# marcinp7/music-style-transfer

Measured on AMD Instinct MI355X. Metric: style-transfer opt iters/sec, higher is better.
Workload: dtype f32; 1 GPU; one 30 s clip per GPU (BASELINE.json configs[1]): piano-roll C=4,R=16,T=4 (+percussion), full widths (980325 params), fwd+loss+bwd every step, Adam+StepLR every iter_size steps; clips_per_gpu=1, iter_size=2, hip_graph=True, graphs=one joint graph, accumulation=2 concurrent streams, launches_per_pass=71, parallelism=single GPU

## Files before the change

include/mst_amd.h:

```cpp
#ifndef MST_AMD_H
#define MST_AMD_H
#include <stdint.h>

#ifdef __cplusplus
extern "C" {
#endif

typedef enum {
    MST_OK = 0,
    MST_ERR_ARG = -1,
    MST_ERR_UNSUPPORTED = -2,
    MST_ERR_LAUNCH = -3,
    MST_ERR_ALLOC = -4,
} mst_status;

typedef struct {
    int32_t C, R, T;
    int32_t beat, bar, nrf;
    int32_t style, melody, rhythm;
    int32_t instr;
    int32_t n_instruments;
    int32_t has_unpitched;
    int32_t clips;
} mst_dims;
// ... 6 lines not shown
    MST_L_U_TOTAL, MST_L_U_NOTES, MST_L_U_VELOCITY, MST_L_U_DURATION,
    MST_L_SI_TOTAL, MST_L_SI_INSTRUMENTS, MST_L_SI_MODE, MST_L_SI_BPM,
    MST_N_LOSSES
};

typedef struct mst_plan mst_plan;
typedef void* mst_stream;

int32_t mst_param_count(const mst_dims* d);
int64_t mst_param_floats(const mst_dims* d);
int32_t mst_param_info(const mst_dims* d, int32_t i, char* name, int32_t name_cap,
                       int64_t* offset, int32_t* ndim, int32_t shape[3]);

int32_t mst_widths_supported(const mst_dims* d);

typedef struct {
    int32_t gemm_tile;
    int32_t no_merge;
    int32_t gemm_run;
    int32_t tile_r0, tile_rows;
    int32_t lstm_flavour;
    int32_t dense_flavour;
    int32_t branches;
} mst_plan_options;
mst_plan* mst_plan_create(const mst_dims* d, int32_t* status);
mst_plan* mst_plan_create_ex(const mst_dims* d, const mst_plan_options* opt, int32_t* status);
int32_t mst_plan_gemm_tile(const mst_plan* p);
void mst_plan_destroy(mst_plan* p);
int64_t mst_plan_workspace_floats(const mst_plan* p);
int32_t mst_plan_tensor(const mst_plan* p, const char* name, int64_t* off, int64_t* goff, int64_t* numel);
int32_t mst_plan_launch_count(const mst_plan* p, int32_t stage_mask, int32_t backward);
int32_t mst_plan_layout(const mst_plan* p, int64_t out[4]);

enum { MST_DEV_OK = 0, MST_DEV_LSTM_TIMEOUT = 1  };
int32_t mst_plan_status(const mst_plan* p, float* ws, int32_t clear, int32_t* status, mst_stream stream);

int32_t mst_forward(const mst_plan* p, int32_t stage_mask, const float* params, float* ws,
                    const float* pitched, const float* unpitched, mst_stream stream);

int32_t mst_backward(const mst_plan* p, int32_t stage_mask, const float* params, float* gparams,
                     float* ws, const float* pitched, const float* unpitched, mst_stream stream);
int32_t mst_zero_grads(const mst_plan* p, int32_t stage_mask, float* ws, mst_stream stream);
int64_t mst_plan_zero_floats(const mst_plan* p, int32_t stage_mask);

#define MST_LOSS_SAVED 512
int64_t mst_loss_scratch_floats(void);
// ... 80 lines not shown

int32_t mst_plan_step_count(const mst_plan* p, int32_t stage_mask, int32_t backward);
int32_t mst_plan_step_info(const mst_plan* p, int32_t stage_mask, int32_t backward, int32_t* info );
int32_t mst_plan_step_carried(const mst_plan* p, int32_t stage_mask, int32_t backward, int32_t* carried);
int32_t mst_plan_step_riders(const mst_plan* p, int32_t stage_mask, int32_t backward, int32_t* out);
int32_t mst_plan_zero_rides(const mst_plan* p);
int32_t mst_plan_step_carrier(const mst_plan* p, int32_t stage_mask, int32_t backward, int32_t* out);
int32_t mst_plan_set_lstm_small(mst_plan* p, int32_t on);
int32_t mst_plan_step_gemms(const mst_plan* p, int32_t stage_mask, int32_t backward, int32_t step, int32_t* out, int32_t cap);
int32_t mst_plan_time_steps(const mst_plan* p, int32_t stage_mask, int32_t backward, const float* params,
                            float* gparams, float* ws, const float* pitched, const float* unpitched,
                            mst_stream stream, int32_t reps, float* ms, int32_t* kind, double* flops, double* bytes);

typedef struct mst_audio_plan mst_audio_plan;
mst_audio_plan* mst_audio_plan_create(int32_t n_fft , int32_t hop, int64_t n_samples, int32_t* status);
void mst_audio_plan_destroy(mst_audio_plan* p);
int32_t mst_audio_plan_info(const mst_audio_plan* p, int64_t out[6]);
int32_t mst_audio_stft(const mst_audio_plan* p, const float* audio, float* spec, float* mag, mst_stream stream);
int32_t mst_audio_gram(const mst_audio_plan* p, const float* feat, float* gram, float* ws, mst_stream stream);
int32_t mst_audio_style_iteration(const mst_audio_plan* p, float* x, const float* gram_style, float* grad, float* exp_avg,
                                  float* exp_avg_sq, float* state, float* ws, float* loss, double lr, mst_stream stream);

int32_t mst_debug_slab_columns_disjoint(int64_t off_x, int32_t width_x, int64_t off_y, int32_t width_y, int32_t ld);
int64_t mst_debug_gemm_walk(int32_t kind, int32_t as_b, int32_t rows, int32_t K, int32_t k0, int32_t k1, int32_t kd, int32_t ld,
                            int32_t pb, int32_t pc, int32_t oc, int64_t* compared);
int32_t mst_plan_step_gemm_kinds(const mst_plan* p, int32_t stage_mask, int32_t backward, int32_t step, int32_t* out, int32_t cap);

const char* mst_version(void);

#ifdef __cplusplus
}
#endif
#endif
```

music-style-transfer_amd/csrc/gemm.hip:

```cpp
#include "combine_body.h"
#include "lstm_small_body.h"

__device__ __forceinline__ float act_fwd(int act, float z, int col) {
    if (act == ACT_LEAKY) return z > 0.f ? z : z * LEAKY;
    if (act == ACT_SIGOUT) { float s = 1.f / (1.f + expf(-z)); return col == 0 ? 6.f * s : s; }
    if (act == ACT_BPM) { float s = 1.f / (1.f + expf(-z)); return s * 150.f + 50.f; }
    return z;
}

__device__ __forceinline__ float act_bwd(int act, float y, int col) {
    if (act == ACT_LEAKY) return y > 0.f ? 1.f : LEAKY;
    if (act == ACT_SIGOUT) return col == 0 ? y * (1.f - y * (1.f / 6.f)) : y * (1.f - y);
    if (act == ACT_BPM) { float s = (y - 50.f) * (1.f / 150.f); return 150.f * s * (1.f - s); }
    return 1.f;
}

typedef const MST_GLOBAL_AS float* gcptr;
#define GEMM_PAD 1

template <int KIND>
__host__ __device__ __forceinline__ int off_of(const Operand& o, int i, int j, bool& ok) {
    if constexpr (KIND == OPK_DENSE) {
        return i * (int)o.si + j * (int)o.sj;
    } else if constexpr (KIND == OPK_ACTGRAD) {
// ... 154 lines not shown
    if (compared) *compared = seen;
    return bad;
}

extern "C" int64_t mst_debug_gemm_walk(int32_t kind, int32_t as_b, int32_t rows, int32_t K, int32_t k0, int32_t k1, int32_t kd,
                                       int32_t ld, int32_t pb, int32_t pc, int32_t oc, int64_t* compared) {
    if (rows < 1 || K < 1 || k0 < 0 || k0 % 8 || k1 > K || k0 > k1 || (kd != 32 && kd != 64 && kd != 128)) return MST_ERR_ARG;
    Operand o{};
    o.kind = kind; o.ld = ld; o.pb = pb; o.pc = pc; o.oc = oc; o.ones_at = -1;
#define WALK_KD(KIND, ISB, KF, PERM)                                                                      \
    return kd == 32 ? walk_mismatches<KIND, ISB, KF, 32, PERM>(o, rows, k0, k1, compared)                 \
                    : (kd == 64 ? walk_mismatches<KIND, ISB, KF, 64, PERM>(o, rows, k0, k1, compared)     \
                                : walk_mismatches<KIND, ISB, KF, 128, PERM>(o, rows, k0, k1, compared));
    if (kind == OPK_IM2COL && !as_b) { WALK_KD(OPK_IM2COL, false, 1, 0) }
    if (kind == OPK_IM2COL && as_b) { WALK_KD(OPK_IM2COL, true, 0, 0) }
    if (kind == OPK_CONVGRAD && !as_b) { WALK_KD(OPK_CONVGRAD, false, 1, 0) }
    if (kind == OPK_PERMW && as_b && perm_case(pb, pc) == 1) { WALK_KD(OPK_PERMW, true, 1, 1) }
    if (kind == OPK_PERMW && as_b && perm_case(pb, pc) == 2) { WALK_KD(OPK_PERMW, true, 1, 2) }
#undef WALK_KD
    return MST_ERR_UNSUPPORTED;
}

template <int OK>
__device__ __forceinline__ void store_out(const GemmDesc& d, float* cbase, const float* bias, int m, int n, int split, float acc) {
    const OutSpec& o = d.out;
    if constexpr (OK == OUT_STORE) {
        float v = acc;
        if (bias) v += o.bias_div > 0 ? bias[(unsigned)((m / o.bias_div) * o.bias_ld + n)] : bias[n];
        cbase[(unsigned)(m * o.ldc + n)] = act_fwd(o.act, v, n);
    } else if constexpr (OK == OUT_ACCUM) {
        float* c = cbase + (unsigned)(m * o.ldc + n);
        *c = o.first ? acc : *c + acc;
    } else if constexpr (OK == OUT_CONV) {
        cbase[(unsigned)((m >> 3) * o.ldc + n * NOCT + (m & 7))] = act_fwd(ACT_LEAKY, acc + bias[n], 0);
    } else if constexpr (OK == OUT_SLAB) {
        const unsigned idx = n < o.wcols ? (unsigned)(m * o.wcols + n) : (unsigned)(d.M * o.wcols + m);
        cbase[(int64_t)split * o.slab_stride + idx] = acc;
    } else {
        unsigned idx;
        if (n < o.wcols) {
            int a, bb, c, bc;
            if (o.pb == CONV_K && o.pc == NPF) { bc = CONV_K * NPF; a = n / (CONV_K * NPF); const int rem = n - a * (CONV_K * NPF); bb = rem / NPF; c = rem - bb * NPF; }
            else if (o.pb == NUN && o.pc == NUF) { bc = NUN * NUF; a = n / (NUN * NUF); const int rem = n - a * (NUN * NUF); bb = rem / NUF; c = rem - bb * NUF; }
            else { bc = o.pb * o.pc; a = n / bc; const int rem = n - a * bc; bb = rem / o.pc; c = rem - bb * o.pc; }
            idx = (unsigned)(m * o.wcols + a * bc + c * o.pb + bb);
        } else {
            idx = (unsigned)(d.M * o.wcols + m);
        }
        cbase[(int64_t)split * o.slab_stride + idx] = acc;
    }
}

template <int AK, int BKIND, int OK, int AKF, int BKF, int KD, int PERM = 0>
__device__ __forceinline__ void gemm_body(const GemmDesc& d, const Bases& b, const int tile, const int split,
                                          float (*As)[GEMM_BM + GEMM_PAD], float (*Bs)[GEMM_BN + GEMM_PAD]) {
    const int tid = threadIdx.x;
    const int M = d.M, N = d.N;
    const int tiles_n = (N + GEMM_BN - 1) / GEMM_BN;
    const gcptr baseA = (gcptr)(b.p[d.A.space] + d.A.off);
    const gcptr baseA2 = (AK == OPK_ACTGRAD || AK == OPK_CONVGRAD) ? (gcptr)(b.p[d.A.space2] + d.A.off2) : baseA;
    const gcptr baseB = (gcptr)(b.p[d.B.space] + d.B.off);
    const int tm = tile / tiles_n, tn = tile - tm * tiles_n;
    int kchunk = (d.K + d.ksplit - 1) / d.ksplit;
    kchunk = (kchunk + KD - 1) / KD * KD;
    const int k0 = split * kchunk;
    const int k1 = min(d.K, k0 + kchunk);
    const int wv = tid >> 6, lane = tid & 63;
    const int a_act = (AK == OPK_ACTGRAD) ? d.A.act : ACT_LEAKY;
    const int a_tr = d.A.transposed;
    const int b_ones = (BKIND == OPK_DENSE || BKIND == OPK_IM2COL) ? d.B.ones_at : -1;
    typedef float acc_f32x16 __attribute__((ext_vector_type(16)));
// ... 21 lines not shown
            int ia = wa.at(d.A, i, (KT), k1, ina, oka);                                                    \
            ia = oka ? ia : 0;                                                                             \
            const float x = baseA[(unsigned)ia];                                                           \
            if constexpr (AK == OPK_ACTGRAD || AK == OPK_CONVGRAD) {                                       \
                const float y = baseA2[(unsigned)ia];                                                      \
                int col = 0;                                                                               \
                if constexpr (AK == OPK_ACTGRAD) col = a_tr ? tm * GEMM_BM + A_ROW(i) : (KT) + A_KL(i);    \
                ya[i] = act_bwd(a_act, y, col);                                                            \
            } else ya[i] = 1.f;                                                                            \
            va[i] = oka ? x : 0.f;                                                                         \
            bool inb, okb;                                                                                 \
            int ib = wb.at(d.B, i, (KT), k1, inb, okb);                                                    \
            bool one = false;                                                                              \
            if constexpr (BKIND == OPK_DENSE || BKIND == OPK_IM2COL) one = inb & (tn * GEMM_BN + B_ROW(i) == b_ones); \
            ib = (okb & !one) ? ib : 0;                                                                    \
            const float w = baseB[(unsigned)ib];                                                           \
            vb[i] = one ? 1.f : (okb ? w : 0.f);                                                           \
        }                                                                                                  \
        wa.advance();                                                                                      \
        wb.advance();                                                                                      \
    }

    if (k0 < k1) GEMM_ISSUE(k0)
    for (int kt = k0; kt < k1; kt += KD) {
#pragma unroll
        for (int i = 0; i < NL; ++i) {
            As[A_KL(i)][A_ROW(i)] = (AK == OPK_ACTGRAD || AK == OPK_CONVGRAD) ? va[i] * ya[i] : va[i];
            Bs[B_KL(i)][B_ROW(i)] = vb[i];
        }
        __syncthreads();
        if (kt + KD < k1) GEMM_ISSUE(kt + KD)
#pragma unroll
        for (int kk = 0; kk < KW; kk += 2) {
            const int k = wv * KW + kk + (lane >> 5);
            acc = __builtin_amdgcn_mfma_f32_32x32x2f32(As[k][lane & 31], Bs[k][lane & 31], acc, 0, 0, 0);
        }
        __syncthreads();
    }
#undef GEMM_ISSUE
#undef A_ROW
#undef A_KL
#undef B_ROW
#undef B_KL
    float* red = &As[0][0];
#pragma unroll
    for (int r = 0; r < 16; ++r)
        red[wv * (GEMM_BM * GEMM_BN) + ((r & 3) + 8 * (r >> 2) + 4 * (lane >> 5)) * GEMM_BN + (lane & 31)] = acc[r];
    __syncthreads();
    float* cbase = b.p[d.out.space] + d.out.off;
    const float* bias = d.out.bias_space >= 0 ? b.p[d.out.bias_space] + d.out.bias_off : nullptr;
#pragma unroll
    for (int q = 0; q < GEMM_BM * GEMM_BN / NT; ++q) {
        const int o = tid + q * NT;
        const int m = tm * GEMM_BM + o / GEMM_BN, n = tn * GEMM_BN + o % GEMM_BN;
        float v = 0.f;
#pragma unroll
        for (int w = 0; w < NW; ++w) v += red[w * (GEMM_BM * GEMM_BN) + o];
        if (m < M && n < N) store_out<OK>(d, cbase, bias, m, n, split, v);
    }
}

#define MF_BM 64
#define MF_BN 64
#define MF_KD 32
#define MF_THREADS 256
typedef float mf_f32x16 __attribute__((ext_vector_type(16)));
typedef float mf_f4u __attribute__((ext_vector_type(4), aligned(4)));

template <int AK, int BKIND, int OK, int AKF, int BKF, bool FOLD = false>
__device__ __forceinline__ void gemm_mfma_body(const GemmDesc& d, const Bases& b, const int tile, const int split,
                                               float (*As)[MF_BM + GEMM_PAD], float (*Bs)[MF_BN + GEMM_PAD]) {
    const int tid = threadIdx.x;
    const int M = d.M, N = d.N;
    const int tiles_n = (N + MF_BN - 1) / MF_BN;
    const gcptr baseA = (gcptr)(b.p[d.A.space] + d.A.off);
    const gcptr baseA2 = (AK == OPK_ACTGRAD || AK == OPK_CONVGRAD) ? (gcptr)(b.p[d.A.space2] + d.A.off2) : baseA;
    const gcptr baseB = (gcptr)(b.p[d.B.space] + d.B.off);
    const int tm = tile / tiles_n, tn = tile - tm * tiles_n;
    int kchunk = (d.K + d.ksplit - 1) / d.ksplit;
    kchunk = (kchunk + MF_KD - 1) / MF_KD * MF_KD;
// ... 787 lines not shown
```

music-style-transfer_amd/csrc/plan.hip:

```cpp
#include <algorithm>
#include <cmath>
#include <cstdio>
#include <cstdlib>
#include <cstring>
#include <map>
#include <string>
#include <array>
#include <vector>

#include "mst_common.h"

#define MST_ALIGN_UP(n) (((n) + 63) / 64 * 64)

static int mean_size(double a, double b, double factor = 1.0) { return (int)std::ceil(((a + b) / 2.0) * factor); }

Sizes mst_sizes(const mst_dims& d) {
    Sizes z{};
    z.I = d.instr; z.STYLE = d.style; z.BAR = d.bar; z.H = d.beat; z.HB = d.bar / 2; z.RH = d.rhythm;
    z.MEL = d.melody; z.NRF = d.nrf; z.NI = d.n_instruments;
    z.OC = mean_size(NF * NPF, d.beat);
    z.PCE_IL = mean_size(d.instr, d.beat);
    z.SE_L = mean_size(d.bar, d.style);
    z.SE_IL = mean_size(d.instr, d.style, .25);
    z.SE_ML = mean_size(2, d.style, .1);
// ... 202 lines not shown
struct Acc { int space; int64_t lo, hi; bool w; bool accum = false, dense = true; };
struct Op { int stage; std::vector<Step> fwd, bwd; };

static int stage_idx(int stage) { return stage == MST_STAGE_EXTRACT ? 0 : stage == MST_STAGE_INFO ? 1 : 2; }

struct mst_plan {
    mst_dims d; Sizes z; ParamTable pt;
    DescTable<GemmDesc> gemms; DescTable<GatherDesc> gathers; DescTable<SegRedDesc> segreds; DescTable<LstmDesc> lstms;
    DescTable<CombineDesc> combines; DescTable<NotesDesc> notes; DescTable<RowLinDesc> rowlins;
    DescTable<ConvDesc> convs; DescTable<LinDesc> lins; DescTable<CopyDesc> copies; DescTable<FoldDesc> folds;
    std::vector<SlabEntry> slabs[3];
    std::vector<Op> ops;
    std::vector<Step> sched[2];
    std::vector<Step> sched_all[2];
    const std::vector<Step>& list(int mask, int backward) const { return mask == MST_STAGE_ALL ? sched_all[backward ? 1 : 0] : sched[backward ? 1 : 0]; }
    std::vector<int> s_gemm_owner; int* d_gemm_owner = nullptr;
    std::map<std::string, T> named;
    int64_t act_top = 0, tmp_top = 0;
    SlabEntry* d_slabs[3] = {nullptr, nullptr, nullptr};
    std::vector<SlabBlock> slab_blocks[3]; SlabBlock* d_slab_blocks[3] = {nullptr, nullptr, nullptr};
    std::vector<SlabEntry> slabs_all; SlabEntry* d_slabs_all = nullptr;
    std::vector<SlabBlock> slab_blocks_all; SlabBlock* d_slab_blocks_all = nullptr;
    bool slabs_all_ok = false;
    T t_losses, t_saved, t_gl; int64_t loss_scratch = 0;
    struct LossOps { int64_t pp, up, il, mlg, bp, it, mt, bt, losses, saved, gl, np, nu; } loss{};
    void resolve_loss() {
        auto at = [&](const char* n) { return named.at(n).off; };
        const bool U = d.has_unpitched != 0;
        loss = {at("pitched_pred"), U ? at("unpitched_pred") : 0, at("instruments_pred"), at("mode_pred"), at("bpm_pred"),
                at("used_instruments"), at("mode"), at("bpm_target"), t_losses.off, t_saved.off, t_gl.off,
                (int64_t)P() * NF * NPN, U ? (int64_t)Q() * NF * NUN : 0};
    }
    std::vector<ZeroChunk> zero_stage[3], zero_all;
    ZeroChunk* d_zero_stage[3] = {nullptr, nullptr, nullptr}; ZeroChunk* d_zero_all = nullptr;
    int err = 0;
    mst_plan_options opt{};
    int mfma = 0;
    int lstm_small_on = 1;

    bool tiled() const { return opt.tile_rows > 0; }
    bool mixes() const { return !mfma && !tiled() && opt.branches != 1 && !opt.no_merge; }
    int mc4() const { return d.C <= 4 ? 1 : 0; }
    int Rl() const { return tiled() ? opt.tile_rows : d.R; }
    int P() const { return d.C * Rl() * d.T; }
    int Q() const { return Rl() * d.T; }
    struct Xchg { int space; int64_t off; int32_t len; };
// ... 518 lines not shown
        Op op; op.stage = stage;
        if (global && tiled()) {
            const int ci = (int)combines.host.size();
            op.fwd = {Step{K_COMB_F1, ci, 1, c.nblk, 0}, Step{K_COMB_F2, ci, 1, c.nblk, 0}};
            fold_exchange(op.fwd, 1, SP_TMP, c.part_off, c.nblk, COMBINE_MAXC + 1, Cn, 1);
            op.bwd = {Step{K_COMB_B1, ci, 1, c.nblk, 0}, Step{K_COMB_B2, ci, 1, c.nblk, 0}};
            fold_exchange(op.bwd, 1, SP_TMP, c.part_off, c.nblk, COMBINE_MAXC + 1, Cn + 1, 1);
        } else {
            op.fwd.push_back(Step{K_COMB_F, (int)combines.host.size(), 1, c.nblk, large});
            op.bwd.push_back(Step{K_COMB_B, (int)combines.host.size(), 1, c.nblk, large});
        }
        combines.host.push_back(c);
        ops.push_back(op);
    }

    void build();
    void accesses(const Step& s, std::vector<Acc>& out, bool scheduled = false) const;
    void first_writers(std::vector<Step>& list, size_t begin, bool per_stage, std::vector<Acc>& zero);
    void schedule_pass(const std::vector<Step>& seq, std::vector<Step>& out, bool across_stages);
    int ride_slot(const Step& s) const;
    bool assign_streams(std::vector<Step>& L);
    int n_signals = 0;
    void schedule();
    int upload();
};

static const int RS1[4] = {1, 1, 1, 1};

void mst_plan::build() {
    const int C = d.C, R = Rl(), Rt = d.R, r0 = tiled() ? opt.tile_r0 : 0, Tn = d.T, P_ = P(), Q_ = Q();
    const bool TL = tiled();
    const bool U = d.has_unpitched != 0;
    const int E = MST_STAGE_EXTRACT, IN = MST_STAGE_INFO, AP = MST_STAGE_APPLY;
    T instr = newT(C, z.I, "instr"), mode = newT(1, 2, "mode"), bpm = newT(1, 1, "bpm");
    newT(1, z.NI, "used_instruments"); newT(1, 1, "bpm_target");
    status_off = newT(1, 64, "device_status").off;
    t_losses = newT(1, 64, "losses"); t_saved = newT(1, MST_LOSS_SAVED, "loss_saved"); t_gl = newT(1, 64, "grad_losses");
    loss_scratch = tmp(mst_loss_scratch_floats());
    auto seg0 = [&](const T& t) { return seg(t, 0, 0, 0, 0, true); };

    std::string m = "pitched_channels_encoder";
    T pce_il = linear(E, instr, false, m + ".instruments_linear", z.PCE_IL, ACT_LEAKY);
    T x1 = conv(E);
    const int rsCQ[4] = {C, R * Tn, 1, 1};
    T pcat = gather(E, rsCQ, {seg(x1, R * Tn, 1, 0, 0), seg(pce_il, 1, 0, 0, 0)});
    T pa = linear(E, pcat, true, m + ".linear", z.H, ACT_LEAKY);
// ... 770 lines not shown
    accesses(L[first], acc, true);
    for (const int r : L[first].rider) if (r >= 0) accesses(L[r], acc, true);
    for (const Acc& a : acc) {
        const int64_t ab = arena(a.space);
        if (ab < 0) continue;
        for (int k = 0; k < K(); ++k)
            for (const ZeroChunk& c : zero_all) {
                const int64_t lo = arena(SP_GRAD) + shift(SP_GRAD, k) + c.off;
                if (ab + a.lo < lo + c.len && lo < ab + a.hi) return;
            }
    }
    zero_ride = first;
}

static bool slab_columns_disjoint(int64_t off_x, int width_x, int64_t off_y, int width_y, int ld) {
    const int64_t cx = off_x % ld, cy = off_y % ld;
    if (cx + width_x > ld || cy + width_y > ld) return false;
    return cx + width_x <= cy || cy + width_y <= cx;
}
extern "C" int32_t mst_debug_slab_columns_disjoint(int64_t off_x, int32_t width_x, int64_t off_y, int32_t width_y, int32_t ld) {
    return slab_columns_disjoint(off_x, width_x, off_y, width_y, ld) ? 1 : 0;
}

int mst_plan::upload() {
    int e = 0;
    e |= gemms.upload(); e |= gathers.upload(); e |= segreds.upload(); e |= lstms.upload();
    e |= combines.upload(); e |= notes.upload(); e |= rowlins.upload();
    e |= up(s_gemm_owner, &d_gemm_owner);
    e |= copies.upload(); e |= folds.upload(); e |= up(zero_fwd, &d_zero_fwd);
    for (int st = 0; st < 3; ++st) e |= up(zero_stage[st], &d_zero_stage[st]);
    e |= up(zero_all, &d_zero_all);
    for (int s = 0; s < 3; ++s) {
        for (auto& ent : slabs[s]) { ent.reps = ent.single ? 1 : K(); ent.rep_stride = tmp_top; }
        e |= up(slabs[s], &d_slabs[s]);
        for (size_t i = 0; i < slabs[s].size(); ++i)
            for (int st = 0; st < slabs[s][i].count; st += 64) slab_blocks[s].push_back(SlabBlock{(int)i, st});
        e |= up(slab_blocks[s], &d_slab_blocks[s]);
    }
    {
        std::vector<std::pair<int64_t, int64_t>> spans;
        for (int s = 0; s < 3; ++s)
            for (auto& ent : slabs[s]) {
                const int64_t hi = ent.width > 0 ? ent.dst + (int64_t)(ent.count / ent.width - 1) * ent.dst_ld + ent.width : ent.dst + ent.count;
                spans.push_back({ent.dst, hi});
                slabs_all.push_back(ent);
            }
        slabs_all_ok = true;
        for (size_t i = 0; i < slabs_all.size() && slabs_all_ok; ++i)
            for (size_t j = i + 1; j < slabs_all.size() && slabs_all_ok; ++j) {
                const SlabEntry& x = slabs_all[i]; const SlabEntry& y = slabs_all[j];
                if (spans[i].second <= spans[j].first || spans[j].second <= spans[i].first) continue;
                slabs_all_ok = x.width > 0 && y.width > 0 && x.dst_ld == y.dst_ld && x.base == y.base &&
                               slab_columns_disjoint(x.dst - x.base, x.width, y.dst - y.base, y.width, x.dst_ld);
            }
        for (size_t i = 0; i < slabs_all.size(); ++i)
            for (int st = 0; st < slabs_all[i].count; st += 64) slab_blocks_all.push_back(SlabBlock{(int)i, st});
        e |= up(slabs_all, &d_slabs_all);
        e |= up(slab_blocks_all, &d_slab_blocks_all);
    }
    return e ? MST_ERR_ALLOC : MST_OK;
}

extern "C" int32_t mst_widths_supported(const mst_dims* d) {
    if (!dims_ok(d)) return MST_ERR_ARG;
    return widths_supported(mst_sizes(*d)) ? MST_OK : MST_ERR_UNSUPPORTED;
}

extern "C" mst_plan* mst_plan_create(const mst_dims* d, int32_t* status) { return mst_plan_create_ex(d, nullptr, status); }

extern "C" mst_plan* mst_plan_create_ex(const mst_dims* d, const mst_plan_options* opt, int32_t* status) {
    int32_t dummy; if (!status) status = &dummy;
    if (!dims_ok(d)) { *status = MST_ERR_ARG; return nullptr; }
    if (opt && ((opt->gemm_tile != 0 && opt->gemm_tile != 32 && opt->gemm_tile != 64) || opt->gemm_run < 0 || opt->gemm_run > 64)) { *status = MST_ERR_ARG; return nullptr; }
    if (opt && (opt->lstm_flavour < 0 || opt->lstm_flavour > 2 || opt->dense_flavour < 0 || opt->dense_flavour > 2 || opt->branches < 0 || opt->branches > 1)) { *status = MST_ERR_ARG; return nullptr; }
    if (opt && (opt->tile_rows < 0 || opt->tile_r0 < 0 || (opt->tile_rows > 0 && (opt->tile_r0 + opt->tile_rows > d->R || d->clips > 1)))) {
        *status = MST_ERR_ARG; return nullptr;
    }
    mst_plan* p = new mst_plan();
    if (opt) p->opt = *opt;
    p->d = *d; p->z = mst_sizes(*d);
    if (p->d.clips < 1) p->d.clips = 1;
    build_params(*d, p->z, p->pt);
    p->build();
    if (!p->err) { p->resolve_loss(); p->schedule(); }
    if (p->err) { *status = p->err; delete p; return nullptr; }
    int e = p->upload();
    if (e) { *status = e; mst_plan_destroy(p); return nullptr; }
    *status = MST_OK;
    return p;
}

extern "C" void mst_plan_destroy(mst_plan* p) {
    if (!p) return;
    p->gemms.release(); p->gathers.release(); p->segreds.release(); p->lstms.release(); p->combines.release(); p->notes.release();
    p->rowlins.release(); p->copies.release(); p->folds.release();
    hipFree(p->d_gemm_owner); hipFree(p->d_zero_all); hipFree(p->d_zero_fwd);
    for (int st = 0; st < 3; ++st) hipFree(p->d_zero_stage[st]);
    for (int s = 0; s < 3; ++s) { hipFree(p->d_slabs[s]); hipFree(p->d_slab_blocks[s]); }
    hipFree(p->d_slabs_all); hipFree(p->d_slab_blocks_all);
    for (mst_plan::SideSet& q : p->sides) {
        if (q.ev_fork) hipEventDestroy(q.ev_fork);
        for (int i = 0; i < mst_plan::N_SIDE; ++i) { if (q.ev_join[i]) hipEventDestroy(q.ev_join[i]); if (q.side[i]) hipStreamDestroy(q.side[i]); }
        for (hipEvent_t e : q.ev) if (e) hipEventDestroy(e);
    }
    delete p;
}

extern "C" int64_t mst_plan_workspace_floats(const mst_plan* p) { return p ? (int64_t)p->K() * (2 * p->act_top + p->tmp_top) : MST_ERR_ARG; }

extern "C" int32_t mst_plan_gemm_tile(const mst_plan* p) { return p ? (p->mfma ? 64 : 32) : MST_ERR_ARG; }

extern "C" int32_t mst_plan_layout(const mst_plan* p, int64_t out[4]) {
    if (!p || !out) return MST_ERR_ARG;
    out[0] = p->K(); out[1] = p->act_top; out[2] = p->tmp_top; out[3] = p->arena(SP_GRAD);
    return MST_OK;
}

extern "C" int32_t mst_plan_tensor(const mst_plan* p, const char* name, int64_t* off, int64_t* goff, int64_t* numel) {
    if (!p || !name) return MST_ERR_ARG;
    auto it = p->named.find(name);
    if (it == p->named.end()) return MST_ERR_ARG;
    if (off) *off = it->second.off;
    if (goff) *goff = p->arena(SP_GRAD) + it->second.off;
    if (numel) *numel = (int64_t)it->second.rows * it->second.cols;
    return MST_OK;
}

static std::vector<const Step*> steps_of(const mst_plan* p, int mask, int backward) {
    std::vector<const Step*> steps;
    for (auto& s : p->list(mask, backward)) if (s.stage & mask) steps.push_back(&s);
    return steps;
}

extern "C" int32_t mst_plan_launch_count(const mst_plan* p, int32_t mask, int32_t backward) {
    if (!p) return MST_ERR_ARG;
    int n = 0;
    for (const Step* s : steps_of(p, mask, backward))
// ... 448 lines not shown
        o[0] = g.M; o[1] = g.N; o[2] = g.K; o[3] = g.ksplit; o[4] = g.fold_rows; o[5] = gemm_blocks(g, p->mfma);
    }
    return n;
}

extern "C" int32_t mst_plan_step_gemm_kinds(const mst_plan* p, int32_t mask, int32_t backward, int32_t step, int32_t* out, int32_t cap) {
    if (!p || !out) return MST_ERR_ARG;
    const std::vector<const Step*> steps = steps_of(p, mask, backward);
    if (step < 0 || step >= (int)steps.size()) return MST_ERR_ARG;
    const Step& s = *steps[step];
    if (s.kind != K_GEMM && s.kind != K_GEMM_FOLD) return 0;
    int n = 0;
    for (int q = 0; q < s.b && n < cap; ++q, ++n) {
        const GemmDesc& g = p->gemms.sched[s.first + q];
        out[2 * n] = g.variant; out[2 * n + 1] = p->mfma ? 32 : 32 << g.kdsel;
    }
    return n;
}

extern "C" int32_t mst_plan_time_steps(const mst_plan* p, int32_t mask, int32_t backward, const float* params, float* gparams,
                                       float* ws, const float* pitched, const float* unpitched, mst_stream stream,
                                       int32_t reps, float* ms, int32_t* kind, double* flops, double* bytes) {
    if (!p || !params || !ws || !ms || !kind || !flops || !bytes || reps < 1) return MST_ERR_ARG;
    hipStream_t st = (hipStream_t)stream;
    Bases b = make_bases(p, params, gparams, ws, pitched, unpitched);
    if (backward && !p->tiled()) b.flags = MST_BF_LOSS_FUSED;
    if ((mask & MST_STAGE_ALL) == MST_STAGE_ALL) b.flags |= MST_BF_ALL_STAGES;
    hipEvent_t e0, e1;
    if (hipEventCreate(&e0) != hipSuccess || hipEventCreate(&e1) != hipSuccess) return MST_ERR_ALLOC;
    const std::vector<Step>& L = p->list(mask, backward);
    int idx = 0;
    for (const Step* s : steps_of(p, mask, backward)) {
        float t = 0.f;
        if (s->carrier < 0) {
            run_step(p, L, *s, b, st);
            hipEventRecord(e0, st);
            for (int r = 0; r < reps; ++r) run_step(p, L, *s, b, st);
            hipEventRecord(e1, st);
            hipEventSynchronize(e1);
            hipEventElapsedTime(&t, e0, e1);
        }
        ms[idx] = t / reps; kind[idx] = s->kind == K_GEMM_FOLD ? K_GEMM : s->kind;
        step_cost(p, *s, &flops[idx], &bytes[idx]);
        ++idx;
    }
    hipEventDestroy(e0); hipEventDestroy(e1);
// ... 5 lines not shown
```

music-style-transfer_amd/style/_native.py:

```python
import collections
import ctypes as C
import os

import torch

_HERE = os.path.dirname(os.path.abspath(__file__))
DEFAULT_LIB = os.path.join(os.path.dirname(_HERE), 'libmst_amd.so')

STAGE_EXTRACT, STAGE_INFO, STAGE_APPLY, STAGE_ALL = 1, 2, 4, 7
LOSS_SAVED = 512
LOSS_KEYS = [
    'total', 'channels_loss_total', 'channels_loss_pitched_total', 'channels_loss_pitched_notes_loss',
    'channels_loss_pitched_velocity_loss', 'channels_loss_pitched_duration_loss',
    'channels_loss_pitched_accidentals_loss', 'channels_loss_unpitched_total',
    'channels_loss_unpitched_notes_loss', 'channels_loss_unpitched_velocity_loss',
    'channels_loss_unpitched_duration_loss', 'song_info_loss_total', 'song_info_loss_instruments_loss',
    'song_info_loss_mode_loss', 'song_info_loss_bpm_loss',
]
N_LOSSES = len(LOSS_KEYS)


class MstError(RuntimeError):
    pass


class Dims(C.Structure):
    _fields_ = [(n, C.c_int32) for n in ('C', 'R', 'T', 'beat', 'bar', 'nrf', 'style', 'melody', 'rhythm',
                                         'instr', 'n_instruments', 'has_unpitched', 'clips')]

    def key(self):
        return tuple(getattr(self, n) for n, _ in self._fields_)


class PlanOptions(C.Structure):
    _fields_ = [('gemm_tile', C.c_int32), ('no_merge', C.c_int32), ('gemm_run', C.c_int32), ('tile_r0', C.c_int32),
                ('tile_rows', C.c_int32), ('lstm_flavour', C.c_int32), ('dense_flavour', C.c_int32), ('branches', C.c_int32)]


DEV_LSTM_TIMEOUT = 1
ROLL_NONZERO, ROLL_HARD = 0, 1
WINDOW_WORDS = 4
METRIC_WORDS = 8
ROW_FIELDS = 8
EVAL_ACC_WORDS = 41


class RowFields(C.Structure):
    _fields_ = [('n', C.c_int32), ('src', C.c_int32 * ROW_FIELDS), ('len', C.c_int32 * ROW_FIELDS), ('dst', C.c_int64 * ROW_FIELDS)]

    @classmethod
    def of(cls, fields):
        fields = list(fields)
        if not 1 <= len(fields) <= ROW_FIELDS:
            raise MstError(f'mst_row_fields holds 1 to {ROW_FIELDS} fields, not {len(fields)}')
        out = cls(n=len(fields))
        for f, (src, n, dst) in enumerate(fields):
            out.src[f], out.len[f], out.dst[f] = int(src), int(n), int(dst)
        return out

# ... 15 lines not shown
        raise MstError(f'MST_GEMM={ge!r}: expected mfma or valu')
    return dict(gemm_tile={'mfma': 64, 'valu': 32}.get(ge, 0), no_merge=int(bool(os.environ.get('MST_NO_MERGE'))),
                gemm_run=int(os.environ.get('MST_GEMM_RUN', '0')), lstm_flavour=int(os.environ.get('MST_LSTM_FLAVOUR', '0')),
                dense_flavour=int(os.environ.get('MST_DENSE_FLAVOUR', '0')), branches=int(os.environ.get('MST_BRANCHES', '0')))


_P = C.c_void_p
_SIGS = {
    'mst_param_count': (C.c_int32, [C.POINTER(Dims)]),
    'mst_param_floats': (C.c_int64, [C.POINTER(Dims)]),
    'mst_param_info': (C.c_int32, [C.POINTER(Dims), C.c_int32, C.c_char_p, C.c_int32, C.POINTER(C.c_int64),
                                   C.POINTER(C.c_int32), C.POINTER(C.c_int32 * 3)]),
    'mst_widths_supported': (C.c_int32, [C.POINTER(Dims)]),
    'mst_plan_create': (_P, [C.POINTER(Dims), C.POINTER(C.c_int32)]),
    'mst_plan_create_ex': (_P, [C.POINTER(Dims), C.POINTER(PlanOptions), C.POINTER(C.c_int32)]),
    'mst_plan_gemm_tile': (C.c_int32, [_P]),
    'mst_plan_destroy': (None, [_P]),
    'mst_plan_workspace_floats': (C.c_int64, [_P]),
    'mst_plan_tensor': (C.c_int32, [_P, C.c_char_p, C.POINTER(C.c_int64), C.POINTER(C.c_int64), C.POINTER(C.c_int64)]),
    'mst_plan_launch_count': (C.c_int32, [_P, C.c_int32, C.c_int32]),
    'mst_plan_layout': (C.c_int32, [_P, C.POINTER(C.c_int64 * 4)]),
    'mst_plan_status': (C.c_int32, [_P, _P, C.c_int32, C.POINTER(C.c_int32), _P]),
    'mst_debug_slab_columns_disjoint': (C.c_int32, [C.c_int64, C.c_int32, C.c_int64, C.c_int32, C.c_int32]),
    'mst_forward': (C.c_int32, [_P, C.c_int32, _P, _P, _P, _P, _P]),
    'mst_backward': (C.c_int32, [_P, C.c_int32, _P, _P, _P, _P, _P, _P]),
    'mst_zero_grads': (C.c_int32, [_P, C.c_int32, _P, _P]),
    'mst_plan_zero_floats': (C.c_int64, [_P, C.c_int32]),
    'mst_loss_scratch_floats': (C.c_int64, []),
    'mst_total_loss_fwd': (C.c_int32, [_P, _P, C.c_int64, _P, _P, C.c_int64, _P, _P, C.c_int32, _P, _P, _P, _P,
                                       C.c_int32, _P, _P, _P, _P]),
    'mst_total_loss_bwd': (C.c_int32, [_P, _P, C.c_int64, _P, _P, C.c_int64, _P, _P, C.c_int32, _P, _P, _P, _P,
                                       _P, _P, _P, _P, _P, _P, _P, _P]),
    'mst_train_iteration': (C.c_int32, [_P, _P, _P, _P, _P, _P, _P, _P]),
    'mst_tiled_phase_count': (C.c_int32, [_P]),
    'mst_tiled_phase': (C.c_int32, [_P, C.c_int32, _P, _P, _P, _P, _P, _P, C.c_int32, _P, C.POINTER(C.c_int64 * 8), C.POINTER(C.c_int64 * 8),
                        C.POINTER(C.c_int32)]),
    'mst_adam_step': (C.c_int32, [_P, _P, _P, _P, C.c_int64, _P, C.c_double, C.c_double, C.c_double, C.c_double,
                                  C.c_int32, C.c_double, C.c_int32, _P]),
    'mst_adam_step2': (C.c_int32, [_P, _P, _P, _P, _P, C.c_int64, _P, C.c_double, C.c_double, C.c_double, C.c_double,
                                   C.c_int32, C.c_double, C.c_int32, _P]),
    'mst_grad_guard_scratch_bytes': (C.c_int64, [C.c_int64]),
    'mst_grad_norm': (C.c_int32, [_P, _P, C.c_int64, _P, _P, _P]),
    'mst_grad_norms': (C.c_int32, [_P, _P, _P, _P, C.c_int32, _P, _P]),
    'mst_adam_step_guarded': (C.c_int32, [_P, _P, _P, _P, _P, C.c_int64, _P, _P, _P, C.c_double, C.c_double, C.c_double, C.c_double,
                                          C.c_int32, C.c_double, C.c_double, C.c_int32, C.c_int32, _P]),
    'mst_hard_output': (C.c_int32, [_P, _P, C.c_int64, C.c_int32, _P]),
# ... 124 lines not shown
              'mst_eval_accumulate')

    def plan(self, dims, device):
        opts = options_from_env()
        key = (dims.key(), str(device), tuple(sorted(opts.items())))
        if key in self._plans:
            self._plans.move_to_end(key)
            return self._plans[key]
        plan = self._plans[key] = Plan(self, dims, device, **opts)
        while len(self._plans) > max(1, self._plan_cap):
            self._plans.popitem(last=False)
        return plan


def current_stream(device):
    if torch.device(device).type == 'cuda':
        return torch.cuda.current_stream(device).cuda_stream
    return None


class Plan:
    WS_POOL_CAP = 4

    def __init__(self, native, dims, device, gemm_tile=None, no_merge=None, gemm_run=None, tile_r0=0, tile_rows=0, lstm_flavour=None, dense_flavour=None, branches=None):
        self.native, self.lib, self.dims, self.device = native, native.lib, dims, torch.device(device)
        env = options_from_env()
        opts = PlanOptions(gemm_tile=env['gemm_tile'] if gemm_tile is None else gemm_tile,
                           no_merge=env['no_merge'] if no_merge is None else int(no_merge),
                           gemm_run=env['gemm_run'] if gemm_run is None else int(gemm_run), tile_r0=int(tile_r0), tile_rows=int(tile_rows),
                           lstm_flavour=env['lstm_flavour'] if lstm_flavour is None else int(lstm_flavour),
                           dense_flavour=env['dense_flavour'] if dense_flavour is None else int(dense_flavour),
                           branches=env['branches'] if branches is None else int(branches))
        st = C.c_int32()
        self.handle = self.lib.mst_plan_create_ex(C.byref(dims), C.byref(opts), C.byref(st))
        if not self.handle:
            check(st.value or -1, 'mst_plan_create_ex')
        self.gemm_tile = self.lib.mst_plan_gemm_tile(self.handle)
        self.branches = bool(opts.branches)
        n = self.lib.mst_plan_workspace_floats(self.handle)
        self.ws = torch.zeros(n, dtype=torch.float32, device=self.device)
        self._free_ws = []
        self._touched = {}
        self._slots = {}
        lay = (C.c_int64 * 4)()
        check(self.lib.mst_plan_layout(self.handle, C.byref(lay)), 'mst_plan_layout')
        self.clips, self.clip_stride = int(lay[0]), int(lay[1])

    def __del__(self):
        try:
            if getattr(self, 'handle', None):
                self.lib.mst_plan_destroy(self.handle)
                self.handle = None
        except Exception:
            pass

# ... 34 lines not shown

    def status(self, ws=None, clear=True):
        word = C.c_int32()
        check(self.lib.mst_plan_status(self.handle, ptr(self.ws if ws is None else ws), int(bool(clear)), C.byref(word),
                                       current_stream(self.device)), 'mst_plan_status')
        return word.value

    def check_status(self, ws=None):
        word = self.status(ws)
        if word:
            raise MstError('device status: ' + describe_status(word))

    def _touch(self, ws):
        if self.branches and self.device.type == 'cuda' and torch.cuda.is_current_stream_capturing():
            raise MstError('a plan made with branches=1 cannot run under torch.cuda.graph capture; capture needs branches=0')
        ws = self.ws if ws is None else ws
        self._touched[id(ws)] = ws
        return ws

    def check_touched(self):
        touched, self._touched = self._touched, {}
        for ws in touched.values():
            self.check_status(ws)

    def launch_count(self, mask=STAGE_ALL, backward=False):
        return self.lib.mst_plan_launch_count(self.handle, mask, int(backward))

    def forward(self, mask, params, pitched, unpitched, ws=None):
        check(self.lib.mst_forward(self.handle, mask, ptr(params), ptr(self._touch(ws)), ptr(pitched),
                                   ptr(unpitched), current_stream(self.device)), 'mst_forward')

    def backward(self, mask, params, gparams, pitched, unpitched, ws=None):
        check(self.lib.mst_backward(self.handle, mask, ptr(params), ptr(gparams), ptr(self._touch(ws)),
                                    ptr(pitched), ptr(unpitched), current_stream(self.device)), 'mst_backward')

    def zero_grads(self, mask, ws=None):
        check(self.lib.mst_zero_grads(self.handle, mask, ptr(self.ws if ws is None else ws), current_stream(self.device)),
              'mst_zero_grads')

    def time_steps(self, mask, backward, params, gparams, pitched, unpitched, reps=20):
        import numpy as np
        n = self.lib.mst_plan_step_count(self.handle, mask, int(backward))
        ms, kind = np.zeros(n, np.float32), np.zeros(n, np.int32)
        fl, by = np.zeros(n, np.float64), np.zeros(n, np.float64)
        got = self.lib.mst_plan_time_steps(self.handle, mask, int(backward), ptr(params), ptr(gparams), ptr(self.ws),
                                           ptr(pitched), ptr(unpitched), current_stream(self.device), reps,
# ... 107 lines not shown
```

Baseline: 2908 iters/s.

## Write single-producer weight-gradient GEMM outputs directly into gradient buffer

For weight-gradient GEMMs whose slab output has exactly one producer (no k-split), the plan now points the GEMM epilogue straight at the parameter-gradient arena and removes the matching slab-reduction entries. The kernel reads the old gradient value before the k-loop and writes old+acc directly, so no intermediate slab write or later reduction pass is needed for those outputs. This cuts workspace traffic and slab-reduction work, at the cost of an extra gradient load per lane and an option flag (slab_direct=1 disables it). Some accumulation-ordering and aliasing assumptions now rest on the disjointness check being run before scheduling.

```diff
diff --git a/include/mst_amd.h b/include/mst_amd.h
--- a/include/mst_amd.h
+++ b/include/mst_amd.h
@@ -52,6 +52,7 @@
     int32_t lstm_flavour;
     int32_t dense_flavour;
     int32_t branches;
+    int32_t slab_direct;
 } mst_plan_options;
 mst_plan* mst_plan_create(const mst_dims* d, int32_t* status);
 mst_plan* mst_plan_create_ex(const mst_dims* d, const mst_plan_options* opt, int32_t* status);
@@ -178,6 +179,7 @@
                                   float* exp_avg_sq, float* state, float* ws, float* loss, double lr, mst_stream stream);
 
 int32_t mst_debug_slab_columns_disjoint(int64_t off_x, int32_t width_x, int64_t off_y, int32_t width_y, int32_t ld);
+int32_t mst_plan_slab_info(const mst_plan* p, int64_t out[4]);
 int64_t mst_debug_gemm_walk(int32_t kind, int32_t as_b, int32_t rows, int32_t K, int32_t k0, int32_t k1, int32_t kd, int32_t ld,
                             int32_t pb, int32_t pc, int32_t oc, int64_t* compared);
 int32_t mst_plan_step_gemm_kinds(const mst_plan* p, int32_t stage_mask, int32_t backward, int32_t step, int32_t* out, int32_t cap);
diff --git a/music-style-transfer_amd/csrc/gemm.hip b/music-style-transfer_amd/csrc/gemm.hip
--- a/music-style-transfer_amd/csrc/gemm.hip
+++ b/music-style-transfer_amd/csrc/gemm.hip
@@ -200,6 +200,17 @@
 }
 
 template <int OK>
+__device__ __forceinline__ int slab_col(const OutSpec& o, int n) {
+    if constexpr (OK == OUT_PERMW_SLAB) {
+        int a, bb, c, bc;
+        if (o.pb == CONV_K && o.pc == NPF) { bc = CONV_K * NPF; a = n / (CONV_K * NPF); const int rem = n - a * (CONV_K * NPF); bb = rem / NPF; c = rem - bb * NPF; }
+        else if (o.pb == NUN && o.pc == NUF) { bc = NUN * NUF; a = n / (NUN * NUF); const int rem = n - a * (NUN * NUF); bb = rem / NUF; c = rem - bb * NUF; }
+        else { bc = o.pb * o.pc; a = n / bc; const int rem = n - a * bc; bb = rem / o.pc; c = rem - bb * o.pc; }
+        return a * bc + c * o.pb + bb;
+    } else return n;
+}
+
+template <int OK>
 __device__ __forceinline__ void store_out(const GemmDesc& d, float* cbase, const float* bias, int m, int n, int split, float acc) {
     const OutSpec& o = d.out;
     if constexpr (OK == OUT_STORE) {
@@ -211,20 +222,8 @@
         *c = o.first ? acc : *c + acc;
     } else if constexpr (OK == OUT_CONV) {
         cbase[(unsigned)((m >> 3) * o.ldc + n * NOCT + (m & 7))] = act_fwd(ACT_LEAKY, acc + bias[n], 0);
-    } else if constexpr (OK == OUT_SLAB) {
-        const unsigned idx = n < o.wcols ? (unsigned)(m * o.wcols + n) : (unsigned)(d.M * o.wcols + m);
-        cbase[(int64_t)split * o.slab_stride + idx] = acc;
     } else {
-        unsigned idx;
-        if (n < o.wcols) {
-            int a, bb, c, bc;
-            if (o.pb == CONV_K && o.pc == NPF) { bc = CONV_K * NPF; a = n / (CONV_K * NPF); const int rem = n - a * (CONV_K * NPF); bb = rem / NPF; c = rem - bb * NPF; }
-            else if (o.pb == NUN && o.pc == NUF) { bc = NUN * NUF; a = n / (NUN * NUF); const int rem = n - a * (NUN * NUF); bb = rem / NUF; c = rem - bb * NUF; }
-            else { bc = o.pb * o.pc; a = n / bc; const int rem = n - a * bc; bb = rem / o.pc; c = rem - bb * o.pc; }
-            idx = (unsigned)(m * o.wcols + a * bc + c * o.pb + bb);
-        } else {
-            idx = (unsigned)(d.M * o.wcols + m);
-        }
+        const unsigned idx = n < o.wcols ? (unsigned)(m * o.wcols + slab_col<OK>(o, n)) : (unsigned)(d.M * o.wcols + m);
         cbase[(int64_t)split * o.slab_stride + idx] = acc;
     }
 }
@@ -292,6 +291,18 @@
     }
 
     if (k0 < k1) GEMM_ISSUE(k0)
+    static_assert(GEMM_BM * GEMM_BN == GEMM_THREADS, "one output element per lane");
+    constexpr bool SLAB = OK == OUT_SLAB || OK == OUT_PERMW_SLAB;
+    constexpr int NO_ELEM = -0x7fffffff - 1;
+    int goff = NO_ELEM;
+    float gold = 0.f;
+    if constexpr (SLAB) {
+        const int m = tm * GEMM_BM + tid / GEMM_BN, n = tn * GEMM_BN + tid % GEMM_BN;
+        if (d.out.first && m < M && n < N) {
+            goff = n < d.out.wcols ? m * d.out.ldc + slab_col<OK>(d.out, n) : (int)(d.out.bias_off - d.out.off) + m;
+            gold = ((gcptr)(b.p[SP_GPAR] + d.out.off))[goff];
+        }
+    }
     for (int kt = k0; kt < k1; kt += KD) {
 #pragma unroll
         for (int i = 0; i < NL; ++i) {
@@ -326,6 +337,12 @@
         float v = 0.f;
 #pragma unroll
         for (int w = 0; w < NW; ++w) v += red[w * (GEMM_BM * GEMM_BN) + o];
+        if constexpr (SLAB) {
+            if (d.out.first) {
+                if (goff != NO_ELEM) cbase[goff] = gold + (v + 0.f);
+                continue;
+            }
+        }
         if (m < M && n < N) store_out<OK>(d, cbase, bias, m, n, split, v);
     }
 }
diff --git a/music-style-transfer_amd/csrc/plan.hip b/music-style-transfer_amd/csrc/plan.hip
--- a/music-style-transfer_amd/csrc/plan.hip
+++ b/music-style-transfer_amd/csrc/plan.hip
@@ -248,6 +248,7 @@
     std::vector<SlabEntry> slabs_all; SlabEntry* d_slabs_all = nullptr;
     std::vector<SlabBlock> slab_blocks_all; SlabBlock* d_slab_blocks_all = nullptr;
     bool slabs_all_ok = false;
+    int64_t direct_elems = 0;
     T t_losses, t_saved, t_gl; int64_t loss_scratch = 0;
     struct LossOps { int64_t pp, up, il, mlg, bp, it, mt, bt, losses, saved, gl, np, nu; } loss{};
     void resolve_loss() {
@@ -812,6 +813,7 @@
     bool assign_streams(std::vector<Step>& L);
     int n_signals = 0;
     void schedule();
+    void redirect_single_producers();
     int upload();
 };
 
@@ -1628,6 +1630,50 @@
     return slab_columns_disjoint(off_x, width_x, off_y, width_y, ld) ? 1 : 0;
 }
 
+void mst_plan::redirect_single_producers() {
+    {
+        std::vector<SlabEntry> all;
+        std::vector<std::pair<int64_t, int64_t>> spans;
+        for (int s = 0; s < 3; ++s)
+            for (auto& ent : slabs[s]) {
+                const int64_t hi = ent.width > 0 ? ent.dst + (int64_t)(ent.count / ent.width - 1) * ent.dst_ld + ent.width : ent.dst + ent.count;
+                spans.push_back({ent.dst, hi});
+                all.push_back(ent);
+            }
+        slabs_all_ok = true;
+        for (size_t i = 0; i < all.size() && slabs_all_ok; ++i)
+            for (size_t j = i + 1; j < all.size() && slabs_all_ok; ++j) {
+                const SlabEntry& x = all[i]; const SlabEntry& y = all[j];
+                if (spans[i].second <= spans[j].first || spans[j].second <= spans[i].first) continue;
+                slabs_all_ok = x.width > 0 && y.width > 0 && x.dst_ld == y.dst_ld && x.base == y.base &&
+                               slab_columns_disjoint(x.dst - x.base, x.width, y.dst - y.base, y.width, x.dst_ld);
+            }
+    }
+    if (opt.slab_direct || !slabs_all_ok || K() != 1 || mfma_plan() || pt.top > 0x7FFFFFFF) return;
+    for (GemmDesc& g : gemms.host) {
+        OutSpec& o = g.out;
+        if ((o.kind != OUT_SLAB && o.kind != OUT_PERMW_SLAB) || g.ksplit != 1 || g.fold_rows) continue;
+        const int64_t wsrc = o.off, bsrc = o.off + (int64_t)g.M * o.wcols;
+        int64_t dir_w = -1, dir_b = -1;
+        int dir_ld = 0;
+        for (int s = 0; s < 3; ++s) {
+            auto& v = slabs[s];
+            for (size_t i = 0; i < v.size();) {
+                const SlabEntry& e = v[i];
+                if (e.splits == 1 && e.src == wsrc && e.count == g.M * o.wcols) {
+                    dir_w = e.dst; dir_ld = e.width > 0 ? e.dst_ld : o.wcols;
+                } else if (e.splits == 1 && e.src == bsrc && e.count == g.M && g.N == o.wcols + 1) {
+                    dir_b = e.dst;
+                } else { ++i; continue; }
+                direct_elems += e.count;
+                v.erase(v.begin() + i);
+            }
+        }
+        if (dir_w < 0 || (g.N == o.wcols + 1) != (dir_b >= 0)) { err = MST_ERR_UNSUPPORTED; return; }
+        o.first = 1; o.space = SP_GPAR; o.off = dir_w; o.ldc = dir_ld; o.bias_off = dir_b >= 0 ? dir_b : dir_w;
+    }
+}
+
 int mst_plan::upload() {
     int e = 0;
     e |= gemms.upload(); e |= gathers.upload(); e |= segreds.upload(); e |= lstms.upload();
@@ -1643,27 +1689,11 @@
             for (int st = 0; st < slabs[s][i].count; st += 64) slab_blocks[s].push_back(SlabBlock{(int)i, st});
         e |= up(slab_blocks[s], &d_slab_blocks[s]);
     }
-    {
-        std::vector<std::pair<int64_t, int64_t>> spans;
-        for (int s = 0; s < 3; ++s)
-            for (auto& ent : slabs[s]) {
-                const int64_t hi = ent.width > 0 ? ent.dst + (int64_t)(ent.count / ent.width - 1) * ent.dst_ld + ent.width : ent.dst + ent.count;
-                spans.push_back({ent.dst, hi});
-                slabs_all.push_back(ent);
-            }
-        slabs_all_ok = true;
-        for (size_t i = 0; i < slabs_all.size() && slabs_all_ok; ++i)
-            for (size_t j = i + 1; j < slabs_all.size() && slabs_all_ok; ++j) {
-                const SlabEntry& x = slabs_all[i]; const SlabEntry& y = slabs_all[j];
-                if (spans[i].second <= spans[j].first || spans[j].second <= spans[i].first) continue;
-                slabs_all_ok = x.width > 0 && y.width > 0 && x.dst_ld == y.dst_ld && x.base == y.base &&
-                               slab_columns_disjoint(x.dst - x.base, x.width, y.dst - y.base, y.width, x.dst_ld);
-            }
-        for (size_t i = 0; i < slabs_all.size(); ++i)
-            for (int st = 0; st < slabs_all[i].count; st += 64) slab_blocks_all.push_back(SlabBlock{(int)i, st});
-        e |= up(slabs_all, &d_slabs_all);
-        e |= up(slab_blocks_all, &d_slab_blocks_all);
-    }
+    for (int s = 0; s < 3; ++s) slabs_all.insert(slabs_all.end(), slabs[s].begin(), slabs[s].end());
+    for (size_t i = 0; i < slabs_all.size(); ++i)
+        for (int st = 0; st < slabs_all[i].count; st += 64) slab_blocks_all.push_back(SlabBlock{(int)i, st});
+    e |= up(slabs_all, &d_slabs_all);
+    e |= up(slab_blocks_all, &d_slab_blocks_all);
     return e ? MST_ERR_ALLOC : MST_OK;
 }
 
@@ -1678,7 +1708,7 @@
     int32_t dummy; if (!status) status = &dummy;
     if (!dims_ok(d)) { *status = MST_ERR_ARG; return nullptr; }
     if (opt && ((opt->gemm_tile != 0 && opt->gemm_tile != 32 && opt->gemm_tile != 64) || opt->gemm_run < 0 || opt->gemm_run > 64)) { *status = MST_ERR_ARG; return nullptr; }
-    if (opt && (opt->lstm_flavour < 0 || opt->lstm_flavour > 2 || opt->dense_flavour < 0 || opt->dense_flavour > 2 || opt->branches < 0 || opt->branches > 1)) { *status = MST_ERR_ARG; return nullptr; }
+    if (opt && (opt->lstm_flavour < 0 || opt->lstm_flavour > 2 || opt->dense_flavour < 0 || opt->dense_flavour > 2 || opt->branches < 0 || opt->branches > 1 || opt->slab_direct < 0 || opt->slab_direct > 1)) { *status = MST_ERR_ARG; return nullptr; }
     if (opt && (opt->tile_rows < 0 || opt->tile_r0 < 0 || (opt->tile_rows > 0 && (opt->tile_r0 + opt->tile_rows > d->R || d->clips > 1)))) {
         *status = MST_ERR_ARG; return nullptr;
     }
@@ -1688,6 +1718,7 @@
     if (p->d.clips < 1) p->d.clips = 1;
     build_params(*d, p->z, p->pt);
     p->build();
+    if (!p->err) p->redirect_single_producers();
     if (!p->err) { p->resolve_loss(); p->schedule(); }
     if (p->err) { *status = p->err; delete p; return nullptr; }
     int e = p->upload();
@@ -1719,6 +1750,17 @@
 extern "C" int32_t mst_plan_layout(const mst_plan* p, int64_t out[4]) {
     if (!p || !out) return MST_ERR_ARG;
     out[0] = p->K(); out[1] = p->act_top; out[2] = p->tmp_top; out[3] = p->arena(SP_GRAD);
+    return MST_OK;
+}
+
+extern "C" int32_t mst_plan_slab_info(const mst_plan* p, int64_t out[4]) {
+    if (!p || !out) return MST_ERR_ARG;
+    int64_t left = 0, blocks = 0;
+    for (int s = 0; s < 3; ++s) {
+        for (const SlabEntry& e : p->slabs[s]) left += e.count;
+        blocks += (int64_t)p->slab_blocks[s].size();
+    }
+    out[0] = p->direct_elems; out[1] = left; out[2] = blocks; out[3] = p->slabs_all_ok ? 1 : 0;
     return MST_OK;
 }
 
@@ -2213,6 +2255,7 @@
                                        float* ws, const float* pitched, const float* unpitched, mst_stream stream,
                                        int32_t reps, float* ms, int32_t* kind, double* flops, double* bytes) {
     if (!p || !params || !ws || !ms || !kind || !flops || !bytes || reps < 1) return MST_ERR_ARG;
+    if (backward && !gparams && p->direct_elems) return MST_ERR_ARG;
     hipStream_t st = (hipStream_t)stream;
     Bases b = make_bases(p, params, gparams, ws, pitched, unpitched);
     if (backward && !p->tiled()) b.flags = MST_BF_LOSS_FUSED;
diff --git a/music-style-transfer_amd/style/_native.py b/music-style-transfer_amd/style/_native.py
--- a/music-style-transfer_amd/style/_native.py
+++ b/music-style-transfer_amd/style/_native.py
@@ -34,7 +34,8 @@
 
 class PlanOptions(C.Structure):
     _fields_ = [('gemm_tile', C.c_int32), ('no_merge', C.c_int32), ('gemm_run', C.c_int32), ('tile_r0', C.c_int32),
-                ('tile_rows', C.c_int32), ('lstm_flavour', C.c_int32), ('dense_flavour', C.c_int32), ('branches', C.c_int32)]
+                ('tile_rows', C.c_int32), ('lstm_flavour', C.c_int32), ('dense_flavour', C.c_int32), ('branches', C.c_int32),
+                ('slab_direct', C.c_int32)]
 
 
 DEV_LSTM_TIMEOUT = 1
@@ -96,6 +97,7 @@
     'mst_plan_layout': (C.c_int32, [_P, C.POINTER(C.c_int64 * 4)]),
     'mst_plan_status': (C.c_int32, [_P, _P, C.c_int32, C.POINTER(C.c_int32), _P]),
     'mst_debug_slab_columns_disjoint': (C.c_int32, [C.c_int64, C.c_int32, C.c_int64, C.c_int32, C.c_int32]),
+    'mst_plan_slab_info': (C.c_int32, [_P, C.POINTER(C.c_int64 * 4)]),
     'mst_forward': (C.c_int32, [_P, C.c_int32, _P, _P, _P, _P, _P]),
     'mst_backward': (C.c_int32, [_P, C.c_int32, _P, _P, _P, _P, _P, _P]),
     'mst_zero_grads': (C.c_int32, [_P, C.c_int32, _P, _P]),
@@ -266,7 +268,7 @@
 class Plan:
     WS_POOL_CAP = 4
 
-    def __init__(self, native, dims, device, gemm_tile=None, no_merge=None, gemm_run=None, tile_r0=0, tile_rows=0, lstm_flavour=None, dense_flavour=None, branches=None):
+    def __init__(self, native, dims, device, gemm_tile=None, no_merge=None, gemm_run=None, tile_r0=0, tile_rows=0, lstm_flavour=None, dense_flavour=None, branches=None, slab_direct=0):
         self.native, self.lib, self.dims, self.device = native, native.lib, dims, torch.device(device)
         env = options_from_env()
         opts = PlanOptions(gemm_tile=env['gemm_tile'] if gemm_tile is None else gemm_tile,
@@ -274,7 +276,7 @@
                            gemm_run=env['gemm_run'] if gemm_run is None else int(gemm_run), tile_r0=int(tile_r0), tile_rows=int(tile_rows),
                            lstm_flavour=env['lstm_flavour'] if lstm_flavour is None else int(lstm_flavour),
                            dense_flavour=env['dense_flavour'] if dense_flavour is None else int(dense_flavour),
-                           branches=env['branches'] if branches is None else int(branches))
+                           branches=env['branches'] if branches is None else int(branches), slab_direct=int(slab_direct))
         st = C.c_int32()
         self.handle = self.lib.mst_plan_create_ex(C.byref(dims), C.byref(opts), C.byref(st))
         if not self.handle:
@@ -355,6 +357,11 @@
         touched, self._touched = self._touched, {}
         for ws in touched.values():
             self.check_status(ws)
+
+    def slab_info(self):
+        out = (C.c_int64 * 4)()
+        check(self.lib.mst_plan_slab_info(self.handle, C.byref(out)), 'mst_plan_slab_info')
+        return tuple(int(v) for v in out)
 
     def launch_count(self, mask=STAGE_ALL, backward=False):
         return self.lib.mst_plan_launch_count(self.handle, mask, int(backward))
```

Result: no change. 2935 iters/s (median of 6 runs) (+1.0%).
